# chathurawidanage/harp

Measured on AMD Instinct MI355X. Metric: sec/iteration K-means (N=1e8, d=100, K=1e4), lower is better.
Workload: dtype bf16; 1 GPU; model=kmeans-allreduce, N=100000000, d=100, K=10000, global_batch=100000000, parallelism=dp1

## Files before the change

csrc/kmeans_resolve.hip:

```cpp
#include "common.h"

namespace {

constexpr int KR_RUN = 2048;

template <int KS>
__global__ __launch_bounds__(64) __attribute__((amdgpu_waves_per_eu(3))) void kmeans_resolve_rowsum_kernel(
    const __bf16* __restrict__ X, long ldx, const __bf16* __restrict__ Cm2, const int* __restrict__ perm,
    const int* __restrict__ start, int NG, long n, int* __restrict__ labels, float* __restrict__ sums, int ld) {
  constexpr int DP = KS * 16;
  constexpr int NCB = (DP + 31) / 32;
  constexpr int STRE = NCB * 32 + 8;
  __shared__ __attribute__((aligned(16))) __bf16 tile[32 * STRE];
  __shared__ bf16x8 atile[KS * 64];
  const int lane = threadIdx.x;
  const int c = lane & 31, h = lane >> 5;
  const long j0 = (long)blockIdx.x * KR_RUN;
  if (j0 >= n) return;
  const long j1 = j0 + KR_RUN < n ? j0 + KR_RUN : n;

  for (int i = lane; i < 32 * STRE; i += 64) tile[i] = (__bf16)0.f;
  int lo = 0, hi = NG;
  while (hi - lo > 1) {
    const int mid = (lo + hi) >> 1;
    if (start[mid] <= j0) lo = mid; else hi = mid;
  }
  int k = lo;
  long kend = start[k + 1];
  int kloaded = -1;
  bool dirty = false;
  floatx16 S[NCB];
#pragma unroll
  for (int b = 0; b < NCB; ++b)
#pragma unroll
    for (int q = 0; q < 16; ++q) S[b][q] = 0.f;

  auto pos = [&](long jb) {
    const long j = jb + c;
    return j < j1 ? j : j1 - 1;
  };
  auto load_rows = [&](bf16x8 (&xf)[KS], int p) {
    const bf16x8* row = (const bf16x8*)(X + (long)p * ldx);
#pragma unroll
    for (int s = 0; s < KS; ++s) xf[s] = row[2 * s + h];
  };
  auto flush = [&](int kk) {
    float* o = sums + ((long)kk * 32 + 4 * h) * ld + c;
#pragma unroll
    for (int b = 0; b < NCB; ++b) {
#pragma unroll
      for (int q = 0; q < 16; ++q) {
        const int rq = (q & 3) + 8 * (q >> 2);
        if (32 * b + c < DP && S[b][q] != 0.f) atomicAdd(o + (long)rq * ld + 32 * b, S[b][q]);
        S[b][q] = 0.f;
      }
    }
  };

  bf16x8 xp[KS];
  int pp = perm[pos(j0)];
  int pn = perm[pos(j0 + 32)];
  load_rows(xp, pp);

  for (long jb = j0; jb < j1; jb += 32) {
    const long je = jb + 32 < j1 ? jb + 32 : j1;
    const long jj = jb + c;
    __syncthreads();
#pragma unroll
    for (int s = 0; s < KS; ++s) *(bf16x8*)(tile + c * STRE + (2 * s + h) * 8) = xp[s];
    const int pc = pp;
    if (jb + 32 < j1) load_rows(xp, pn);
    pp = pn;
    pn = perm[pos(jb + 64)];
    __syncthreads();
    long cur = jb;
    while (cur < je) {
      while (cur >= kend) {
        if (dirty) {
          flush(k);
          dirty = false;
        }
        ++k;
        kend = start[k + 1];
      }
      if (k != kloaded) {
        const bf16x8* arow = (const bf16x8*)(Cm2 + ((long)k * 32 + c) * DP);
#pragma unroll
        for (int s = 0; s < KS; ++s) atile[s * 64 + lane] = arow[2 * s + h];
        kloaded = k;
      }
      const long sub_end = kend < je ? kend : je;
      const bool mine = jj >= cur && jj < sub_end;
      floatx16 acc = {0.f, 0.f, 0.f, 0.f, 0.f, 0.f, 0.f, 0.f, 0.f, 0.f, 0.f, 0.f, 0.f, 0.f, 0.f, 0.f};
#pragma unroll
      for (int s = 0; s < KS; ++s) {
        acc = __builtin_amdgcn_mfma_f32_32x32x16_bf16(atile[s * 64 + lane],
                                                      *(const bf16x8*)(tile + c * STRE + (2 * s + h) * 8), acc, 0, 0, 0);
        __builtin_amdgcn_sched_barrier(0);
      }
      float m = acc[0];
      int mq = 0;
#pragma unroll
      for (int q = 1; q < 16; ++q)
        if (acc[q] < m) {
          m = acc[q];
          mq = q;
        }
      int row = (mq & 3) + 8 * (mq >> 2) + 4 * h;
      const float om = __shfl_xor(m, 32, 64);
      const int orow = __shfl_xor(row, 32, 64);
      if (om < m || (om == m && orow < row)) row = orow;
      if (mine && h == 0) labels[pc] = k * 32 + row;
      const int code = mine ? row : -1;
#pragma unroll
      for (int t = 0; t < 2; ++t) {
        bf16x8 oh;
#pragma unroll
        for (int j = 0; j < 8; ++j) {
          const int r0 = __builtin_amdgcn_readlane(code, 16 * t + j), r1 = __builtin_amdgcn_readlane(code, 16 * t + 8 + j);
          oh[j] = (__bf16)((h ? r1 : r0) == c ? 1.f : 0.f);
        }
        const __bf16* tp = tile + (16 * t + 8 * h) * STRE + c;
#pragma unroll
        for (int b = 0; b < NCB; ++b) {
          bf16x8 xt;
#pragma unroll
          for (int j = 0; j < 8; ++j) xt[j] = tp[j * STRE + 32 * b];
          S[b] = __builtin_amdgcn_mfma_f32_32x32x16_bf16(oh, xt, S[b], 0, 0, 0);
          __builtin_amdgcn_sched_barrier(0);
        }
      }
      dirty = true;
      cur = sub_end;
    }
  }
  if (dirty) flush(k);
}

template <int KS>
int launch_resolve(const void* X, long ldx, const void* Cm2, const int* perm, const int* start, int NG, long n,
                   int* labels, float* sums, int ld, hipStream_t s) {
  const long nblk = (n + KR_RUN - 1) / KR_RUN;
  kmeans_resolve_rowsum_kernel<KS><<<dim3((unsigned)nblk), dim3(64), 0, s>>>(
      (const __bf16*)X, ldx, (const __bf16*)Cm2, perm, start, NG, n, labels, sums, ld);
  return harp_launch_status();
}

}

HARP_EXPORT int harp_kmeans_resolve_rowsum(const void* X, long ldx, const void* Cm2, int dp, const int* perm,
                                           const int* start, int NG, long n, int* labels, float* sums, int ld,
                                           hipStream_t s) {
  if (n <= 0) return n == 0 ? HARP_OK : HARP_EBADARG;
  if (dp <= 0 || dp % 16 || dp > 128 || ldx < dp || ldx % 8 || ld < dp || NG <= 0 || !labels || !sums)
    return HARP_EBADARG;
  switch (dp / 16) {
    case 1: return launch_resolve<1>(X, ldx, Cm2, perm, start, NG, n, labels, sums, ld, s);
    case 2: return launch_resolve<2>(X, ldx, Cm2, perm, start, NG, n, labels, sums, ld, s);
    case 3: return launch_resolve<3>(X, ldx, Cm2, perm, start, NG, n, labels, sums, ld, s);
    case 4: return launch_resolve<4>(X, ldx, Cm2, perm, start, NG, n, labels, sums, ld, s);
    case 5: return launch_resolve<5>(X, ldx, Cm2, perm, start, NG, n, labels, sums, ld, s);
    case 6: return launch_resolve<6>(X, ldx, Cm2, perm, start, NG, n, labels, sums, ld, s);
    case 7: return launch_resolve<7>(X, ldx, Cm2, perm, start, NG, n, labels, sums, ld, s);
    case 8: return launch_resolve<8>(X, ldx, Cm2, perm, start, NG, n, labels, sums, ld, s);
    default: return HARP_EUNSUPPORTED;
  }
}
```

csrc/segsum.hip:

```cpp
#include "common.h"

namespace {

constexpr int SEG = 64;

__global__ __launch_bounds__(256) void label_hist_kernel(const int* __restrict__ lab, long n, int K, long chunk,
                                                         int* __restrict__ H) {
  extern __shared__ __attribute__((aligned(16))) int hist[];
  for (int k = threadIdx.x; k < K; k += blockDim.x) hist[k] = 0;
  __syncthreads();
  const long a = (long)blockIdx.x * chunk;
  long b = a + chunk;
  if (b > n) b = n;
  for (long i = a + threadIdx.x; i < b; i += blockDim.x) atomicAdd(&hist[lab[i]], 1);
  __syncthreads();
  int* row = H + (long)blockIdx.x * K;
  for (int k = threadIdx.x; k < K; k += blockDim.x) row[k] = hist[k];
}

__global__ void colscan1_kernel(int* __restrict__ H, int nchunks, int K, int* __restrict__ T) {
  const int k = blockIdx.x * blockDim.x + threadIdx.x;
  const int s = blockIdx.y;
  if (k >= K) return;
  const int c0 = s * SEG;
  int c1 = c0 + SEG;
  if (c1 > nchunks) c1 = nchunks;
  int run = 0;
  for (int c = c0; c < c1; ++c) {
    const int v = H[(long)c * K + k];
    H[(long)c * K + k] = run;
    run += v;
  }
  T[(long)s * K + k] = run;
}

__global__ void colscan2_kernel(int* __restrict__ T, int nseg, int K, int* __restrict__ counts) {
  const int k = blockIdx.x * blockDim.x + threadIdx.x;
  if (k >= K) return;
  int run = 0;
  for (int s = 0; s < nseg; ++s) {
    const int v = T[(long)s * K + k];
    T[(long)s * K + k] = run;
    run += v;
  }
  counts[k] = run;
}

__global__ __launch_bounds__(1024) void segscan_kernel(const int* __restrict__ counts, int K, int* __restrict__ start) {
  __shared__ int part[1024];
  const int per = (K + 1023) / 1024;
  const int a = threadIdx.x * per;
  int s = 0;
  for (int j = 0; j < per; ++j)
    if (a + j < K) s += counts[a + j];
  part[threadIdx.x] = s;
  __syncthreads();
  for (int off = 1; off < 1024; off <<= 1) {
    const int v = threadIdx.x >= off ? part[threadIdx.x - off] : 0;
    __syncthreads();
    part[threadIdx.x] += v;
    __syncthreads();
  }
  int run = threadIdx.x ? part[threadIdx.x - 1] : 0;
  for (int j = 0; j < per; ++j)
    if (a + j < K) {
      start[a + j] = run;
      run += counts[a + j];
    }
  if (threadIdx.x == 1023) start[K] = part[1023];
}

__device__ __forceinline__ int xcd_contiguous(unsigned b, unsigned nb) {
  const unsigned q = nb / 8, r = nb % 8, x = b % 8;
  return (int)((x < r ? x * (q + 1) : r * (q + 1) + (x - r) * q) + b / 8);
}

__global__ __launch_bounds__(256) void bucket_kernel(const int* __restrict__ lab, long n, int K, long chunk,
                                                     const int* __restrict__ H, const int* __restrict__ T,
                                                     const int* __restrict__ start, int* __restrict__ perm) {
  extern __shared__ __attribute__((aligned(16))) int cur[];
  const int c = xcd_contiguous(blockIdx.x, gridDim.x), s = c / SEG;
  for (int k = threadIdx.x; k < K; k += blockDim.x)
    cur[k] = start[k] + T[(long)s * K + k] + H[(long)c * K + k];
  __syncthreads();
  const long a = (long)c * chunk;
  long b = a + chunk;
  if (b > n) b = n;
  constexpr int U = 8;
  for (long i0 = a + threadIdx.x; i0 < b; i0 += (long)U * blockDim.x) {
    int l[U];
#pragma unroll
    for (int u = 0; u < U; ++u) {
      const long i = i0 + (long)u * blockDim.x;
      l[u] = i < b ? lab[i] : -1;
    }
#pragma unroll
    for (int u = 0; u < U; ++u)
      if (l[u] >= 0) perm[atomicAdd(&cur[l[u]], 1)] = (int)(i0 + (long)u * blockDim.x);
  }
}

template <int LPR, int RUN, int ROWS = 4>
__global__ __launch_bounds__(256) void rowsum_bf16_kernel(const __bf16* __restrict__ X, int dp, long ldx,
                                                          const int* __restrict__ perm,
                                                          const int* __restrict__ start, int K, long n,
                                                          float* __restrict__ sums, int ld) {
  constexpr int SPW = 64 / LPR;
  const int lane = threadIdx.x & 63;
  const int sl = lane % LPR;
  const long slot = ((long)blockIdx.x * blockDim.x + threadIdx.x) / LPR;
  const long j0 = slot * RUN;
  if (j0 >= n) return;
  long j1 = j0 + RUN;
  if (j1 > n) j1 = n;
  const bool active = sl * 8 < dp;
  int lo = 0, hi = K;
  while (hi - lo > 1) {
    const int mid = (lo + hi) >> 1;
    if (start[mid] <= j0) lo = mid; else hi = mid;
  }
  int k = lo;
  long kend = start[k + 1];
  float acc[8] = {0.f, 0.f, 0.f, 0.f, 0.f, 0.f, 0.f, 0.f};
  auto flush = [&](int kk) {
    if (active) {
      float* o = sums + (long)kk * ld + sl * 8;
#pragma unroll
      for (int e = 0; e < 8; ++e) {
        if (acc[e] != 0.f) atomicAdd(o + e, acc[e]);
        acc[e] = 0.f;
      }
    }
  };
  long j = j0;
  while (j < j1) {
    while (j >= kend) {
      flush(k);
      ++k;
      kend = start[k + 1];
    }
    long stop = kend < j1 ? kend : j1;
    for (; j + ROWS <= stop; j += ROWS) {
      bf16x8 v[ROWS];
      int pj[ROWS];
#pragma unroll
      for (int q = 0; q < ROWS; ++q) pj[q] = perm[j + q];
#pragma unroll
      for (int q = 0; q < ROWS; ++q) v[q] = active ? *(const bf16x8*)(X + (long)pj[q] * ldx + sl * 8) : bf16x8{};
#pragma unroll
      for (int q = 0; q < ROWS; q += 4)
#pragma unroll
        for (int e = 0; e < 8; ++e)
          acc[e] += ((float)v[q][e] + (float)v[q + 1][e]) + ((float)v[q + 2][e] + (float)v[q + 3][e]);
    }
    for (; j < stop; ++j) {
      if (active) {
        const bf16x8 v = *(const bf16x8*)(X + (long)perm[j] * ldx + sl * 8);
#pragma unroll
        for (int e = 0; e < 8; ++e) acc[e] += (float)v[e];
      }
    }
  }
  flush(k);
  (void)SPW;
}

template <int VEC, int RUN, int ROWS = 4>
__global__ __launch_bounds__(256) void rowsum_wide_bf16_kernel(const __bf16* __restrict__ X, int dp, long ldx,
                                                               const int* __restrict__ perm,
                                                               const int* __restrict__ start, int K, long n,
                                                               float* __restrict__ sums, int ld) {
  const int lane = threadIdx.x & 63;
  const long slot = ((long)blockIdx.x * blockDim.x + threadIdx.x) >> 6;
  const long j0 = slot * RUN;
  if (j0 >= n) return;
  long j1 = j0 + RUN;
  if (j1 > n) j1 = n;
  bool active[VEC];
#pragma unroll
  for (int c = 0; c < VEC; ++c) active[c] = (64 * c + lane) * 8 < dp;
  int lo = 0, hi = K;
  while (hi - lo > 1) {
    const int mid = (lo + hi) >> 1;
    if (start[mid] <= j0) lo = mid; else hi = mid;
  }
  int k = lo;
  long kend = start[k + 1];
  float acc[VEC][8];
#pragma unroll
  for (int c = 0; c < VEC; ++c)
#pragma unroll
    for (int e = 0; e < 8; ++e) acc[c][e] = 0.f;
  auto flush = [&](int kk) {
#pragma unroll
    for (int c = 0; c < VEC; ++c) {
      if (active[c]) {
        float* o = sums + (long)kk * ld + (64 * c + lane) * 8;
#pragma unroll
        for (int e = 0; e < 8; ++e) {
          if (acc[c][e] != 0.f) atomicAdd(o + e, acc[c][e]);
          acc[c][e] = 0.f;
        }
      }
    }
  };
  long j = j0;
  while (j < j1) {
    while (j >= kend) {
      flush(k);
      ++k;
      kend = start[k + 1];
    }
    const long stop = kend < j1 ? kend : j1;
    for (; j + ROWS <= stop; j += ROWS) {
      int pj[ROWS];
#pragma unroll
      for (int q = 0; q < ROWS; ++q) pj[q] = perm[j + q];
      bf16x8 v[ROWS][VEC];
#pragma unroll
      for (int q = 0; q < ROWS; ++q)
#pragma unroll
        for (int c = 0; c < VEC; ++c)
          v[q][c] = active[c] ? *(const bf16x8*)(X + (long)pj[q] * ldx + (64 * c + lane) * 8) : bf16x8{};
#pragma unroll
      for (int c = 0; c < VEC; ++c)
#pragma unroll
        for (int q = 0; q < ROWS; q += 4)
#pragma unroll
          for (int e = 0; e < 8; ++e)
            acc[c][e] += ((float)v[q][c][e] + (float)v[q + 1][c][e]) + ((float)v[q + 2][c][e] + (float)v[q + 3][c][e]);
    }
    for (; j < stop; ++j) {
      const long r = perm[j];
#pragma unroll
      for (int c = 0; c < VEC; ++c) {
        if (active[c]) {
          const bf16x8 v = *(const bf16x8*)(X + r * ldx + (64 * c + lane) * 8);
#pragma unroll
          for (int e = 0; e < 8; ++e) acc[c][e] += (float)v[e];
        }
      }
    }
  }
  flush(k);
}

}

HARP_EXPORT long harp_bucket_chunk(long n) {
  long c = 65536;
  while (c > 4096 && (n + c - 1) / c < 1536) c >>= 1;
  return c;
}

HARP_EXPORT long harp_bucket_workspace_ints(long n, int K) {
  const long chunk = harp_bucket_chunk(n);
  const long nch = (n + chunk - 1) / chunk;
  const long nseg = (nch + SEG - 1) / SEG;
  return nch * K + nseg * K + K + (K + 1) + n;
}

HARP_EXPORT int harp_bucket_labels(const int* lab, long n, int K, int* ws, long* start_off, long* perm_off,
                                   hipStream_t s) {
  if (n <= 0 || K <= 0 || K > 16384) return HARP_EBADARG;
  const long chunk = harp_bucket_chunk(n);
  const int nch = (int)((n + chunk - 1) / chunk);
  const int nseg = (nch + SEG - 1) / SEG;
  int* H = ws;
  int* T = H + (long)nch * K;
  int* counts = T + (long)nseg * K;
  int* start = counts + K;
  int* perm = start + K + 1;
  *start_off = start - ws;
  *perm_off = perm - ws;
  const size_t lds = (size_t)K * sizeof(int);
  label_hist_kernel<<<dim3(nch), dim3(256), lds, s>>>(lab, n, K, chunk, H);
  colscan1_kernel<<<dim3((K + 255) / 256, nseg), dim3(256), 0, s>>>(H, nch, K, T);
  colscan2_kernel<<<dim3((K + 255) / 256), dim3(256), 0, s>>>(T, nseg, K, counts);
  segscan_kernel<<<dim3(1), dim3(1024), 0, s>>>(counts, K, start);
  bucket_kernel<<<dim3(nch), dim3(256), lds, s>>>(lab, n, K, chunk, H, T, start, perm);
  return harp_launch_status();
}

HARP_EXPORT int harp_bucket_rowsum_bf16(const void* X, int dp, long ldx, const int* perm, const int* start, int K,
                                        long n, float* sums, int ld, hipStream_t s) {
  if (dp % 8 || dp > 1024 || ld < dp || ldx < dp || ldx % 8 || n <= 0) return n == 0 ? HARP_OK : HARP_EBADARG;
  const int lpr_min = dp / 8;
  const __bf16* Xb = (const __bf16*)X;
  constexpr int RUN = 256;
  auto grid = [&](int lpr) { return dim3((unsigned)(((n + RUN - 1) / RUN * lpr + 255) / 256)); };
  if (lpr_min <= 8) rowsum_bf16_kernel<8, RUN><<<grid(8), dim3(256), 0, s>>>(Xb, dp, ldx, perm, start, K, n, sums, ld);
  else if (lpr_min <= 16) rowsum_bf16_kernel<16, RUN, 8><<<grid(16), dim3(256), 0, s>>>(Xb, dp, ldx, perm, start, K, n, sums, ld);
  else if (lpr_min <= 32) rowsum_bf16_kernel<32, RUN><<<grid(32), dim3(256), 0, s>>>(Xb, dp, ldx, perm, start, K, n, sums, ld);
  else if (dp <= 512) rowsum_wide_bf16_kernel<1, RUN><<<grid(64), dim3(256), 0, s>>>(Xb, dp, ldx, perm, start, K, n, sums, ld);
  else rowsum_wide_bf16_kernel<2, RUN><<<grid(64), dim3(256), 0, s>>>(Xb, dp, ldx, perm, start, K, n, sums, ld);
  return harp_launch_status();
}
```

harp_amd/ops/_lib.py:

```python
from __future__ import annotations

import ctypes
import os
import threading

import torch

from .build import KERNEL_LIB, RUNTIME_LIB

_lock = threading.Lock()
_kern = None
_rt = None

c_int, c_long, c_float, c_void_p, c_ulonglong, c_double = (
    ctypes.c_int, ctypes.c_long, ctypes.c_float, ctypes.c_void_p, ctypes.c_ulonglong, ctypes.c_double)

_SIGNATURES = {
    "harp_kmeans_points_per_block": [c_int],
    "harp_kmeans_resident_blocks": [c_int, c_int],
    "harp_kmeans_set_resident_blocks": [c_int],
    "harp_kmeans_assign": [c_void_p, c_long, c_void_p, c_long, c_int, c_int, c_int, c_void_p, c_void_p, c_int,
                           c_void_p, c_void_p, c_int, c_void_p],
    "harp_kmeans_assign_wide": [c_void_p, c_long, c_void_p, c_long, c_int, c_int, c_int, c_int, c_void_p, c_int,
                                c_void_p],
    "harp_kmeans_wide_finish": [c_void_p, c_long, c_void_p, c_void_p, c_void_p, c_void_p],
    "harp_kmeans_normalize": [c_void_p, c_int, c_void_p, c_int, c_int, c_void_p, c_void_p],
    "harp_kmeans_prepare": [c_void_p, c_int, c_int, c_int, c_int, c_void_p, c_void_p, c_void_p],
    "harp_uniform_rows_bf16": [c_void_p, c_long, c_int, c_int, c_float, c_float, c_ulonglong, c_long, c_int,
                               c_void_p],
}


class NativeUnavailable(RuntimeError):
    pass


def _bind(lib, sigs):
    for name, args in sigs.items():
        try:
            fn = getattr(lib, name)
        except AttributeError:
            continue
        fn.argtypes = args
        fn.restype = c_int


def register(signatures: dict) -> None:
    _SIGNATURES.update(signatures)
    if _kern is not None:
        _bind(_kern, signatures)


def kernels():
    global _kern
    if _kern is not None:
        return _kern
    with _lock:
        if _kern is None:
            path = os.environ.get("HARP_KERNEL_LIB", KERNEL_LIB)
            if not os.path.exists(path):
                raise NativeUnavailable(
                    f"{path} not built: run `python -c 'import __graft_entry__ as g; g.build()'` "
                    "or `python -m harp_amd.ops.build`")
            try:
                lib = ctypes.CDLL(path, mode=ctypes.RTLD_GLOBAL)
            except OSError as e:
                raise NativeUnavailable(f"cannot load {path}: {e}") from e
            _bind(lib, _SIGNATURES)
            _kern = lib
    return _kern


def runtime():
    global _rt
    path = os.environ.get("HARP_RUNTIME_LIB", RUNTIME_LIB)
    if _rt is None and os.path.exists(path):
        with _lock:
            if _rt is None:
                _rt = ctypes.CDLL(path)
    return _rt


def available() -> bool:
    try:
        kernels()
        return True
    except NativeUnavailable:
        return False


def stream_ptr(device: torch.device | None = None) -> int:
    return torch.cuda.current_stream(device).cuda_stream


def ptr(t: torch.Tensor | None) -> int | None:
    return None if t is None else t.data_ptr()


def check(status: int, what: str) -> None:
    if status != 0:
        names = {1: "bad argument", 2: "launch failure", 3: "unsupported shape"}
        raise RuntimeError(f"{what}: native kernel returned {status} ({names.get(status, '?')})")


def use_native(t: torch.Tensor) -> bool:
    if t.device.type == "cuda":
        kernels()
        return True
    return False
```

harp_amd/ops/kmeans.py:

```python
from __future__ import annotations

import math
import os
from dataclasses import dataclass
from typing import Optional

import torch

from . import _lib, segment

KP_ALIGN = 128
ONES = 4
DEFAULT_VARIANT = 16
KEYLESS_VARIANT, KEYED_VARIANT = 16, 15
KEYLESS_MAX_DP = 128
RESOLVE_SPAN = 1 << 23


NARROW_MAX_DP = 256
WIDE_ALIGN = 64
WIDE_VARIANT = int(os.environ.get("HARP_KMEANS_WIDE_VARIANT", "0"))


def padded_dim(d: int) -> int:
    dp = (d + ONES + 15) // 16 * 16
    return dp if dp <= NARROW_MAX_DP else (d + ONES + WIDE_ALIGN - 1) // WIDE_ALIGN * WIDE_ALIGN


def padded_k(k: int) -> int:
    return (k + KP_ALIGN - 1) // KP_ALIGN * KP_ALIGN


def row_stride(dp: int) -> int:
    return (dp + 127) // 128 * 128


def pack_points(x: torch.Tensor, device: torch.device | str | None = None) -> torch.Tensor:
    device = torch.device(device) if device is not None else x.device
    n, d = x.shape
    dp = padded_dim(d)
    dt = torch.bfloat16 if device.type == "cuda" else torch.float32
    ld = row_stride(dp) if device.type == "cuda" else dp
    out = torch.zeros((n, ld), dtype=dt, device=device)
    out[:, :d] = x.to(device=device, dtype=dt)
    out[:, d:d + ONES] = 1.0
    return out[:, :dp]


def generate_points(n: int, d: int, lo: float = 0.0, hi: float = 1000.0, seed: int = 0,
                    device: torch.device | str = "cpu", row0: int = 0) -> torch.Tensor:
    device = torch.device(device)
    dp = padded_dim(d)
    if device.type == "cuda" and _lib.use_native(torch.empty(0, device=device)):
        ld = row_stride(dp)
        Xs = torch.empty((n, ld), dtype=torch.bfloat16, device=device)
        _lib.check(_lib.kernels().harp_uniform_rows_bf16(Xs.data_ptr(), n, d, ld, float(lo), float(hi),
                                                         seed & 0xFFFFFFFFFFFFFFFF, row0, 1,
                                                         _lib.stream_ptr(device)), "uniform_rows")
        return Xs[:, :dp]
    g = torch.Generator().manual_seed(seed * 1000003 + row0)
    x = torch.rand((n, d), generator=g, dtype=torch.float32) * (hi - lo) + lo
    return pack_points(x, device)


_SIDE: dict = {}


def pipeline_chunks(n: int, ppb: int) -> int:
    c = int(os.environ.get("HARP_KMEANS_CHUNKS", "1"))
    return max(1, min(c, n // (ppb * 256)))


def _side_stream(dev: torch.device) -> torch.cuda.Stream:
    s = _SIDE.get(dev)
    if s is None:
        s = _SIDE[dev] = torch.cuda.Stream(dev)
    return s


@dataclass
class CentroidOperand:
    Cm2: torch.Tensor
    cn: torch.Tensor
    K: int
    d: int


def prepare(c: torch.Tensor, dp: int, out: Optional[CentroidOperand] = None) -> CentroidOperand:
    K, d = c.shape
    Kp = padded_k(K)
    dev = c.device
    if out is None:
        dt = torch.bfloat16 if dev.type == "cuda" else torch.float32
        out = CentroidOperand(torch.empty((Kp, dp), dtype=dt, device=dev), torch.empty(Kp, dtype=torch.float32, device=dev), K, d)
    if _lib.use_native(c):
        cc = c.contiguous().float()
        _lib.check(_lib.kernels().harp_kmeans_prepare(cc.data_ptr(), K, d, Kp, dp, out.Cm2.data_ptr(),
                                                      out.cn.data_ptr(), _lib.stream_ptr(dev)), "kmeans_prepare")
        return out
    out.Cm2.zero_()
    out.Cm2[:K, :d] = -2.0 * c
    out.cn.fill_(1e38)
    out.cn[:K] = (c.double() ** 2).sum(1).float()
    return out


def resident_blocks(variant: int, dp: int) -> int:
    return _lib.kernels().harp_kmeans_resident_blocks(variant, dp // 16)


def set_resident_blocks(n: int) -> None:
    _lib.check(_lib.kernels().harp_kmeans_set_resident_blocks(n), "kmeans_set_resident_blocks")


def swept_k(op: "CentroidOperand") -> int:
    return min(op.Cm2.shape[0], (op.K + 31) // 32 * 32)


def _check_operands(X, op):
    assert X.dtype == torch.bfloat16 and X.stride(1) == 1 and X.stride(0) % 8 == 0 and op.Cm2.shape[1] == X.shape[1]


def _check_sums(sums, op, dev):
    assert sums.dtype == torch.float32 and sums.shape[1] >= op.d + 1 and sums.is_contiguous()
    assert sums.shape[0] >= op.Cm2.shape[0], "sums needs Kp (padded) rows"
    assert sums.device == dev


def _assign_wide(X, op, sums, labels, want_objective, obj_partial, min_dist):
    n, dp = X.shape
    dev = X.device
    lib = _lib.kernels()
    _check_operands(X, op)
    assert dp % WIDE_ALIGN == 0, f"wide rows need dp % {WIDE_ALIGN} == 0 (pack with padded_dim)"
    keys = torch.full((n,), -1, dtype=torch.int64, device=dev)
    _lib.check(lib.harp_kmeans_assign_wide(X.data_ptr(), X.stride(0), op.Cm2.data_ptr(), n, dp, swept_k(op),
                                           op.Cm2.shape[0], op.d, keys.data_ptr(), WIDE_VARIANT, _lib.stream_ptr(dev)),
               "kmeans_assign_wide")
    nblk = (n + 255) // 256
    if want_objective and (obj_partial is None or obj_partial.numel() < nblk):
        obj_partial = torch.empty(nblk, dtype=torch.float32, device=dev)
    _lib.check(lib.harp_kmeans_wide_finish(keys.data_ptr(), n, labels.data_ptr(),
                                           obj_partial.data_ptr() if want_objective else None,
                                           min_dist.data_ptr() if min_dist is not None else None,
                                           _lib.stream_ptr(dev)), "kmeans_wide_finish")
    if sums is not None:
        _check_sums(sums, op, dev)
        perm, start = segment.bucket_labels(labels, op.Cm2.shape[0])
        segment.bucket_rowsum(X, perm, start, sums)
    obj = obj_partial[:nblk].double().sum() if want_objective else None
    return labels, obj


def assign(X: torch.Tensor, op: CentroidOperand, sums: Optional[torch.Tensor] = None,
           labels: Optional[torch.Tensor] = None, want_objective: bool = True, variant: int = DEFAULT_VARIANT,
           obj_partial: Optional[torch.Tensor] = None, accumulate: str = "bucket",
           min_dist: Optional[torch.Tensor] = None):
    n, dp = X.shape
    dev = X.device
    if labels is None:
        labels = torch.empty(n, dtype=torch.int32, device=dev)
    if _lib.use_native(X):
        lib = _lib.kernels()
        if dp > NARROW_MAX_DP:
            if accumulate == "atomic":
                raise ValueError("accumulate='atomic' is only fused into the narrow kernel (dp <= "
                                 f"{NARROW_MAX_DP}); the wide path (dp = {dp}) accumulates by bucket")
            return _assign_wide(X, op, sums, labels, want_objective, obj_partial, min_dist)
        keyless = (variant == KEYLESS_VARIANT and dp <= KEYLESS_MAX_DP and sums is not None
                   and accumulate == "bucket" and min_dist is None)
        if variant == KEYLESS_VARIANT and not keyless:
            variant = KEYED_VARIANT
        if dp > 128:
            variant = 4
        elif variant in (14, 15) and dp // 16 == 5:
            variant = 13
        ppb = lib.harp_kmeans_points_per_block(variant)
        if ppb <= 0:
            raise ValueError(f"unknown kmeans kernel variant {variant}")
        nblk = (n + ppb - 1) // ppb
        if want_objective and (obj_partial is None or obj_partial.numel() < nblk):
            obj_partial = torch.empty(nblk, dtype=torch.float32, device=dev)
        if sums is not None:
            _check_sums(sums, op, dev)
        _check_operands(X, op)
        fused = sums if accumulate == "atomic" else None
        bucket = sums is not None and fused is None
        chunks = pipeline_chunks(n, ppb) if bucket else 1
        per = max(1, (nblk + chunks - 1) // chunks) * ppb
        side = _side_stream(dev) if chunks > 1 else None
        main = torch.cuda.current_stream(dev)
        for r0 in range(0, n, per):
            r1 = min(n, r0 + per)
            b0 = r0 // ppb
            st = lib.harp_kmeans_assign(X[r0].data_ptr(), X.stride(0), op.Cm2.data_ptr(), r1 - r0, dp,
                                        swept_k(op), op.d,
                                        labels[r0].data_ptr(), _lib.ptr(fused),
                                        fused.stride(0) if fused is not None else 0,
                                        obj_partial[b0].data_ptr() if want_objective else None,
                                        min_dist[r0].data_ptr() if min_dist is not None else None, variant,
                                        _lib.stream_ptr(dev))
            _lib.check(st, "kmeans_assign")
            if not bucket:
                continue

            def bucket_sum(lab, Xc):
                if keyless:
                    for s0 in range(0, lab.numel(), RESOLVE_SPAN):
                        ls, Xs = lab[s0:s0 + RESOLVE_SPAN], Xc[s0:s0 + RESOLVE_SPAN]
                        perm, start = segment.bucket_labels(ls, swept_k(op) // 32)
                        segment.resolve_rowsum(Xs, op.Cm2, perm, start, ls, sums)
                else:
                    perm, start = segment.bucket_labels(lab, op.Cm2.shape[0])
                    segment.bucket_rowsum(Xc, perm, start, sums)

            if side is None:
                bucket_sum(labels, X)
                continue
            side.wait_stream(main)
            with torch.cuda.stream(side):
                bucket_sum(labels[r0:r1], X[r0:r1])
        if side is not None:
            main.wait_stream(side)
        obj = obj_partial[:nblk].double().sum() if want_objective else None
        return labels, obj
    Xf = X.float()
    d = op.d
    x = Xf[:, :d]
    C = -0.5 * op.Cm2[: op.K, :d].float()
    dist = op.cn[: op.K].unsqueeze(0) - 2.0 * (x @ C.t())
    lab = dist.argmin(1)
    labels.copy_(lab.to(labels.dtype))
    if min_dist is not None:
        min_dist.copy_((dist.gather(1, lab[:, None])[:, 0] + (x * x).sum(1)).to(min_dist.dtype))
    if sums is not None:
        sums[:, : d + 1].index_add_(0, lab, Xf[:, : d + 1])
    obj = None
    if want_objective:
        xs = (x.double() ** 2).sum(1)
        obj = (dist.gather(1, lab[:, None])[:, 0].double() + xs).clamp_min(0).sum()
    return labels, obj


def normalize(sums: torch.Tensor, c: torch.Tensor, d: int, counts: Optional[torch.Tensor] = None) -> torch.Tensor:
    Kr = c.shape[0]
    if _lib.use_native(c):
        assert sums.is_contiguous() and c.is_contiguous()
        _lib.check(_lib.kernels().harp_kmeans_normalize(sums.data_ptr(), sums.stride(0), c.data_ptr(), Kr, d,
                                                        _lib.ptr(counts), _lib.stream_ptr(c.device)),
                   "kmeans_normalize")
        return c
    cnt = sums[:, d]
    m = cnt > 0
    c[m] = sums[m, :d] / cnt[m, None]
    if counts is not None:
        counts.copy_(cnt)
    return c
```

harp_amd/ops/segment.py:

```python
from __future__ import annotations

import ctypes
import os
from typing import Dict, Tuple

import torch

from . import _lib

_lib.register({
    "harp_bucket_chunk": [_lib.c_long],
    "harp_bucket_workspace_ints": [_lib.c_long, _lib.c_int],
    "harp_bucket_labels": [_lib.c_void_p, _lib.c_long, _lib.c_int, _lib.c_void_p, _lib.c_void_p, _lib.c_void_p,
                           _lib.c_void_p],
    "harp_bucket_rowsum_bf16": [_lib.c_void_p, _lib.c_int, _lib.c_long, _lib.c_void_p, _lib.c_void_p, _lib.c_int,
                                _lib.c_long, _lib.c_void_p, _lib.c_int, _lib.c_void_p],
    "harp_kmeans_resolve_rowsum": [_lib.c_void_p, _lib.c_long, _lib.c_void_p, _lib.c_int, _lib.c_void_p,
                                   _lib.c_void_p, _lib.c_int, _lib.c_long, _lib.c_void_p, _lib.c_void_p, _lib.c_int,
                                   _lib.c_void_p],
})
_WS: Dict[Tuple, torch.Tensor] = {}


def _lib_ret_long(fn):
    fn.restype = ctypes.c_long
    return fn


def bucket_labels(labels: torch.Tensor, K: int) -> Tuple[torch.Tensor, torch.Tensor]:
    n = labels.numel()
    if not _lib.use_native(labels):
        order = torch.argsort(labels.long(), stable=True)
        counts = torch.bincount(labels.long(), minlength=K)
        start = torch.zeros(K + 1, dtype=torch.int64)
        start[1:] = torch.cumsum(counts, 0)
        return order.to(torch.int32), start.to(torch.int32)
    lib = _lib.kernels()
    _lib_ret_long(lib.harp_bucket_workspace_ints)
    need = lib.harp_bucket_workspace_ints(n, K)
    stream = torch.cuda.current_stream(labels.device).cuda_stream
    key = (labels.device, n, K, stream)
    ws = _WS.get(key)
    if ws is None:
        ws = next((w for k, w in _WS.items() if k[0] == labels.device and k[3] == stream and w.numel() >= need),
                  None)
    if ws is None:
        for k in [k for k in _WS if k[3] == stream]:
            del _WS[k]
        ws = torch.empty(need, dtype=torch.int32, device=labels.device)
        _WS[key] = ws
    so, po = ctypes.c_long(0), ctypes.c_long(0)
    st = lib.harp_bucket_labels(labels.data_ptr(), n, K, ws.data_ptr(), ctypes.byref(so), ctypes.byref(po),
                                _lib.stream_ptr(labels.device))
    _lib.check(st, "bucket_labels")
    return ws[po.value:po.value + n], ws[so.value:so.value + K + 1]


SUM_SLICE = min(1024, max(8, int(os.environ.get("HARP_ROWSUM_SLICE", "1024")) // 8 * 8))


def bucket_rowsum(X: torch.Tensor, perm: torch.Tensor, start: torch.Tensor, out: torch.Tensor) -> torch.Tensor:
    K = start.numel() - 1
    if not _lib.use_native(X):
        idx = torch.repeat_interleave(torch.arange(K), (start[1:] - start[:-1]).long())
        out[:K, : X.shape[1]].index_add_(0, idx, X[perm.long()].float())
        return out
    assert X.dtype == torch.bfloat16 and X.stride(1) == 1 and out.dtype == torch.float32 and out.is_contiguous()
    for c0 in range(0, X.shape[1], SUM_SLICE):
        w = min(SUM_SLICE, X.shape[1] - c0)
        st = _lib.kernels().harp_bucket_rowsum_bf16(X[:, c0:].data_ptr(), w, X.stride(0), perm.data_ptr(),
                                                    start.data_ptr(), K, perm.numel(), out[:, c0:].data_ptr(),
                                                    out.stride(0), _lib.stream_ptr(X.device))
        _lib.check(st, "bucket_rowsum")
    return out


def resolve_rowsum(X: torch.Tensor, Cm2: torch.Tensor, perm: torch.Tensor, start: torch.Tensor,
                   labels: torch.Tensor, out: torch.Tensor) -> torch.Tensor:
    NG = start.numel() - 1
    dp = X.shape[1]
    assert X.dtype == torch.bfloat16 and X.stride(1) == 1 and out.dtype == torch.float32 and out.is_contiguous()
    assert Cm2.dtype == torch.bfloat16 and Cm2.is_contiguous() and Cm2.shape[1] == dp and Cm2.shape[0] >= 32 * NG
    assert out.shape[0] >= 32 * NG and labels.dtype == torch.int32 and labels.is_contiguous()
    assert labels.numel() == perm.numel() == X.shape[0]
    st = _lib.kernels().harp_kmeans_resolve_rowsum(X.data_ptr(), X.stride(0), Cm2.data_ptr(), dp, perm.data_ptr(),
                                                   start.data_ptr(), NG, perm.numel(), labels.data_ptr(),
                                                   out.data_ptr(), out.stride(0), _lib.stream_ptr(X.device))
    _lib.check(st, "kmeans_resolve_rowsum")
    return out
```

Before: 0.1323 s/iter.

## Bucket all spans in one pass and finish labels via rank gather

Replaces the Python loop over fixed-size spans, which launched a separate bucket and resolve pass per span, with one span-aware bucketing pipeline keyed by (span, group) and a single resolve launch. The resolve kernel now writes a per-sorted-position byte (row within group) instead of scattering int32 labels through perm. A new finish kernel gathers that byte by rank to build the final labels. The span size is enlarged so far fewer spans exist. This cuts launch count and repeated per-span histogram work and replaces random int32 label writes with coalesced byte writes. In exchange it adds a rank array write and a separate label-finishing pass.

```diff
diff --git a/csrc/kmeans_resolve.hip b/csrc/kmeans_resolve.hip
--- a/csrc/kmeans_resolve.hip
+++ b/csrc/kmeans_resolve.hip
@@ -7,7 +7,8 @@
 template <int KS>
 __global__ __launch_bounds__(64) __attribute__((amdgpu_waves_per_eu(3))) void kmeans_resolve_rowsum_kernel(
     const __bf16* __restrict__ X, long ldx, const __bf16* __restrict__ Cm2, const int* __restrict__ perm,
-    const int* __restrict__ start, int NG, long n, int* __restrict__ labels, float* __restrict__ sums, int ld) {
+    const int* __restrict__ start, int NG, int NB, long n, unsigned char* __restrict__ rowof,
+    float* __restrict__ sums, int ld) {
   constexpr int DP = KS * 16;
   constexpr int NCB = (DP + 31) / 32;
   constexpr int STRE = NCB * 32 + 8;
@@ -20,14 +21,15 @@
   const long j1 = j0 + KR_RUN < n ? j0 + KR_RUN : n;
 
   for (int i = lane; i < 32 * STRE; i += 64) tile[i] = (__bf16)0.f;
-  int lo = 0, hi = NG;
+  int lo = 0, hi = NB;
   while (hi - lo > 1) {
     const int mid = (lo + hi) >> 1;
     if (start[mid] <= j0) lo = mid; else hi = mid;
   }
   int k = lo;
   long kend = start[k + 1];
-  int kloaded = -1;
+  int g = k % NG;
+  int gloaded = -1;
   bool dirty = false;
   floatx16 S[NCB];
 #pragma unroll
@@ -44,8 +46,8 @@
 #pragma unroll
     for (int s = 0; s < KS; ++s) xf[s] = row[2 * s + h];
   };
-  auto flush = [&](int kk) {
-    float* o = sums + ((long)kk * 32 + 4 * h) * ld + c;
+  auto flush = [&](int gg) {
+    float* o = sums + ((long)gg * 32 + 4 * h) * ld + c;
 #pragma unroll
     for (int b = 0; b < NCB; ++b) {
 #pragma unroll
@@ -58,9 +60,8 @@
   };
 
   bf16x8 xp[KS];
-  int pp = perm[pos(j0)];
+  load_rows(xp, perm[pos(j0)]);
   int pn = perm[pos(j0 + 32)];
-  load_rows(xp, pp);
 
   for (long jb = j0; jb < j1; jb += 32) {
     const long je = jb + 32 < j1 ? jb + 32 : j1;
@@ -68,26 +69,27 @@
     __syncthreads();
 #pragma unroll
     for (int s = 0; s < KS; ++s) *(bf16x8*)(tile + c * STRE + (2 * s + h) * 8) = xp[s];
-    const int pc = pp;
     if (jb + 32 < j1) load_rows(xp, pn);
-    pp = pn;
     pn = perm[pos(jb + 64)];
     __syncthreads();
     long cur = jb;
     while (cur < je) {
-      while (cur >= kend) {
+      if (cur >= kend) {
         if (dirty) {
-          flush(k);
+          flush(g);
           dirty = false;
         }
-        ++k;
-        kend = start[k + 1];
-      }
-      if (k != kloaded) {
-        const bf16x8* arow = (const bf16x8*)(Cm2 + ((long)k * 32 + c) * DP);
+        do {
+          ++k;
+          kend = start[k + 1];
+        } while (cur >= kend);
+        g = k % NG;
+      }
+      if (g != gloaded) {
+        const bf16x8* arow = (const bf16x8*)(Cm2 + ((long)g * 32 + c) * DP);
 #pragma unroll
         for (int s = 0; s < KS; ++s) atile[s * 64 + lane] = arow[2 * s + h];
-        kloaded = k;
+        gloaded = g;
       }
       const long sub_end = kend < je ? kend : je;
       const bool mine = jj >= cur && jj < sub_end;
@@ -110,7 +112,7 @@
       const float om = __shfl_xor(m, 32, 64);
       const int orow = __shfl_xor(row, 32, 64);
       if (om < m || (om == m && orow < row)) row = orow;
-      if (mine && h == 0) labels[pc] = k * 32 + row;
+      if (mine && h == 0) rowof[jj] = (unsigned char)row;
       const int code = mine ? row : -1;
 #pragma unroll
       for (int t = 0; t < 2; ++t) {
@@ -134,35 +136,69 @@
       cur = sub_end;
     }
   }
-  if (dirty) flush(k);
+  if (dirty) flush(g);
 }
 
 template <int KS>
-int launch_resolve(const void* X, long ldx, const void* Cm2, const int* perm, const int* start, int NG, long n,
-                   int* labels, float* sums, int ld, hipStream_t s) {
+int launch_resolve(const void* X, long ldx, const void* Cm2, const int* perm, const int* start, int NG, int NB,
+                   long n, unsigned char* rowof, float* sums, int ld, hipStream_t s) {
   const long nblk = (n + KR_RUN - 1) / KR_RUN;
   kmeans_resolve_rowsum_kernel<KS><<<dim3((unsigned)nblk), dim3(64), 0, s>>>(
-      (const __bf16*)X, ldx, (const __bf16*)Cm2, perm, start, NG, n, labels, sums, ld);
+      (const __bf16*)X, ldx, (const __bf16*)Cm2, perm, start, NG, NB, n, rowof, sums, ld);
   return harp_launch_status();
 }
 
+template <bool VEC>
+__global__ __launch_bounds__(256) void kmeans_finish_labels_kernel(int* __restrict__ labels,
+                                                                   const int* __restrict__ rank,
+                                                                   const unsigned char* __restrict__ rowof, long n) {
+  const long p = ((long)blockIdx.x * 256 + threadIdx.x) * 4;
+  if (p >= n) return;
+  if (VEC && p + 4 <= n) {
+    const int4 r = *(const int4*)(rank + p);
+    int4 l = *(const int4*)(labels + p);
+    l.x = 32 * l.x + rowof[r.x];
+    l.y = 32 * l.y + rowof[r.y];
+    l.z = 32 * l.z + rowof[r.z];
+    l.w = 32 * l.w + rowof[r.w];
+    *(int4*)(labels + p) = l;
+  } else {
+    const long e = p + 4 < n ? p + 4 : n;
+    for (long i = p; i < e; ++i) labels[i] = 32 * labels[i] + rowof[rank[i]];
+  }
+}
+
+}
+
+HARP_EXPORT int harp_kmeans_finish_labels(int* labels, const int* rank, const unsigned char* rowof, long n,
+                                          hipStream_t s) {
+  if (n <= 0) return n == 0 ? HARP_OK : HARP_EBADARG;
+  if (!labels || !rank || !rowof || n >= (1L << 31)) return HARP_EBADARG;
+  const dim3 grid((unsigned)((n + 1023) / 1024));
+  if ((((uintptr_t)labels | (uintptr_t)rank) & 15) == 0)
+    kmeans_finish_labels_kernel<true><<<grid, dim3(256), 0, s>>>(labels, rank, rowof, n);
+  else
+    kmeans_finish_labels_kernel<false><<<grid, dim3(256), 0, s>>>(labels, rank, rowof, n);
+  return harp_launch_status();
 }
 
 HARP_EXPORT int harp_kmeans_resolve_rowsum(const void* X, long ldx, const void* Cm2, int dp, const int* perm,
-                                           const int* start, int NG, long n, int* labels, float* sums, int ld,
-                                           hipStream_t s) {
+                                           const int* start, int NG, int nspans, long n, unsigned char* rowof,
+                                           float* sums, int ld, hipStream_t s) {
   if (n <= 0) return n == 0 ? HARP_OK : HARP_EBADARG;
-  if (dp <= 0 || dp % 16 || dp > 128 || ldx < dp || ldx % 8 || ld < dp || NG <= 0 || !labels || !sums)
+  if (dp <= 0 || dp % 16 || dp > 128 || ldx < dp || ldx % 8 || ld < dp || NG <= 0 || nspans <= 0 ||
+      (long)nspans * NG >= (1L << 30) || n >= (1L << 31) || !rowof || !sums)
     return HARP_EBADARG;
+  const int NB = nspans * NG;
   switch (dp / 16) {
-    case 1: return launch_resolve<1>(X, ldx, Cm2, perm, start, NG, n, labels, sums, ld, s);
-    case 2: return launch_resolve<2>(X, ldx, Cm2, perm, start, NG, n, labels, sums, ld, s);
-    case 3: return launch_resolve<3>(X, ldx, Cm2, perm, start, NG, n, labels, sums, ld, s);
-    case 4: return launch_resolve<4>(X, ldx, Cm2, perm, start, NG, n, labels, sums, ld, s);
-    case 5: return launch_resolve<5>(X, ldx, Cm2, perm, start, NG, n, labels, sums, ld, s);
-    case 6: return launch_resolve<6>(X, ldx, Cm2, perm, start, NG, n, labels, sums, ld, s);
-    case 7: return launch_resolve<7>(X, ldx, Cm2, perm, start, NG, n, labels, sums, ld, s);
-    case 8: return launch_resolve<8>(X, ldx, Cm2, perm, start, NG, n, labels, sums, ld, s);
+    case 1: return launch_resolve<1>(X, ldx, Cm2, perm, start, NG, NB, n, rowof, sums, ld, s);
+    case 2: return launch_resolve<2>(X, ldx, Cm2, perm, start, NG, NB, n, rowof, sums, ld, s);
+    case 3: return launch_resolve<3>(X, ldx, Cm2, perm, start, NG, NB, n, rowof, sums, ld, s);
+    case 4: return launch_resolve<4>(X, ldx, Cm2, perm, start, NG, NB, n, rowof, sums, ld, s);
+    case 5: return launch_resolve<5>(X, ldx, Cm2, perm, start, NG, NB, n, rowof, sums, ld, s);
+    case 6: return launch_resolve<6>(X, ldx, Cm2, perm, start, NG, NB, n, rowof, sums, ld, s);
+    case 7: return launch_resolve<7>(X, ldx, Cm2, perm, start, NG, NB, n, rowof, sums, ld, s);
+    case 8: return launch_resolve<8>(X, ldx, Cm2, perm, start, NG, NB, n, rowof, sums, ld, s);
     default: return HARP_EUNSUPPORTED;
   }
 }
diff --git a/csrc/segsum.hip b/csrc/segsum.hip
--- a/csrc/segsum.hip
+++ b/csrc/segsum.hip
@@ -97,6 +97,74 @@
 #pragma unroll
     for (int u = 0; u < U; ++u)
       if (l[u] >= 0) perm[atomicAdd(&cur[l[u]], 1)] = (int)(i0 + (long)u * blockDim.x);
+  }
+}
+
+
+__global__ void colscan1_spans_kernel(int* __restrict__ H, int nchunks, int K, int seg, int* __restrict__ T) {
+  const int k = blockIdx.y * blockDim.x + threadIdx.x;
+  const int s = blockIdx.x;
+  if (k >= K) return;
+  const int c0 = s * seg;
+  int c1 = c0 + seg;
+  if (c1 > nchunks) c1 = nchunks;
+  int run = 0;
+  for (int c = c0; c < c1; ++c) {
+    const int v = H[(long)c * K + k];
+    H[(long)c * K + k] = run;
+    run += v;
+  }
+  T[(long)s * K + k] = run;
+}
+
+__global__ void colscan2_spans_kernel(int* __restrict__ T, int nseg, int sps, int K, int* __restrict__ counts) {
+  const int k = blockIdx.y * blockDim.x + threadIdx.x;
+  const int sp = blockIdx.x;
+  if (k >= K) return;
+  const int s0 = sp * sps;
+  int s1 = s0 + sps;
+  if (s1 > nseg) s1 = nseg;
+  int run = 0;
+  for (int s = s0; s < s1; ++s) {
+    const int v = T[(long)s * K + k];
+    T[(long)s * K + k] = run;
+    run += v;
+  }
+  counts[(long)sp * K + k] = run;
+}
+
+constexpr int SPAN_TPB = 1024;
+constexpr long SPAN_CHUNK = 16384;
+
+__global__ __launch_bounds__(SPAN_TPB) void bucket_spans_kernel(const int* __restrict__ lab, long n, int K,
+                                                                long chunk, int cps, int seg,
+                                                                const int* __restrict__ H, const int* __restrict__ T,
+                                                                const int* __restrict__ start, int* __restrict__ perm,
+                                                                int* __restrict__ rank) {
+  extern __shared__ __attribute__((aligned(16))) int cur[];
+  const int c = xcd_contiguous(blockIdx.x, gridDim.x), s = c / seg;
+  const int* st = start + (long)(c / cps) * K;
+  for (int k = threadIdx.x; k < K; k += blockDim.x) cur[k] = st[k] + T[(long)s * K + k] + H[(long)c * K + k];
+  __syncthreads();
+  const long a = (long)c * chunk;
+  long b = a + chunk;
+  if (b > n) b = n;
+  constexpr int U = 8;
+  for (long i0 = a + threadIdx.x; i0 < b; i0 += (long)U * blockDim.x) {
+    int l[U];
+#pragma unroll
+    for (int u = 0; u < U; ++u) {
+      const long i = i0 + (long)u * blockDim.x;
+      l[u] = i < b ? lab[i] : -1;
+    }
+#pragma unroll
+    for (int u = 0; u < U; ++u)
+      if (l[u] >= 0) {
+        const long i = i0 + (long)u * blockDim.x;
+        const int j = atomicAdd(&cur[l[u]], 1);
+        perm[j] = (int)i;
+        if (rank) rank[i] = j;
+      }
   }
 }
 
@@ -282,6 +350,65 @@
   return harp_launch_status();
 }
 
+namespace {
+
+struct SpanGeom {
+  long chunk;
+  int nch, cps, seg, nseg, sps, nspans;
+  long nb;
+};
+
+bool span_geom(long n, int K, long span, SpanGeom* g) {
+  if (n <= 0 || n >= (1L << 31) || K <= 0 || K > 16384 || span < 1024 || (span & (span - 1))) return false;
+  if (span > (1L << 31)) span = 1L << 31;
+  long chunk = harp_bucket_chunk(n) < SPAN_CHUNK ? harp_bucket_chunk(n) : SPAN_CHUNK;
+  if (chunk > span) chunk = span;
+  const long cps = span / chunk;
+  const long seg = cps < SEG ? cps : SEG;
+  const long nch = (n + chunk - 1) / chunk;
+  const long nspans = (n + span - 1) / span;
+  if (nspans * K >= (1L << 30)) return false;
+  g->chunk = chunk;
+  g->nch = (int)nch;
+  g->cps = (int)cps;
+  g->seg = (int)seg;
+  g->nseg = (int)((nch + seg - 1) / seg);
+  g->sps = (int)(cps / seg);
+  g->nspans = (int)nspans;
+  g->nb = nspans * K;
+  return true;
+}
+
+}
+
+HARP_EXPORT long harp_bucket_spans_workspace_ints(long n, int K, long span) {
+  SpanGeom g;
+  if (!span_geom(n, K, span, &g)) return 0;
+  return (long)g.nch * K + (long)g.nseg * K + g.nb + (g.nb + 1) + n;
+}
+
+HARP_EXPORT int harp_bucket_labels_spans(const int* lab, long n, int K, long span, int* ws, long* start_off,
+                                         long* perm_off, int* rank, hipStream_t s) {
+  SpanGeom g;
+  if (!lab || !ws || !span_geom(n, K, span, &g)) return HARP_EBADARG;
+  int* H = ws;
+  int* T = H + (long)g.nch * K;
+  int* counts = T + (long)g.nseg * K;
+  int* start = counts + g.nb;
+  int* perm = start + g.nb + 1;
+  *start_off = start - ws;
+  *perm_off = perm - ws;
+  const size_t lds = (size_t)K * sizeof(int);
+  const unsigned kb = (unsigned)((K + 255) / 256);
+  label_hist_kernel<<<dim3(g.nch), dim3(256), lds, s>>>(lab, n, K, g.chunk, H);
+  colscan1_spans_kernel<<<dim3(g.nseg, kb), dim3(256), 0, s>>>(H, g.nch, K, g.seg, T);
+  colscan2_spans_kernel<<<dim3(g.nspans, kb), dim3(256), 0, s>>>(T, g.nseg, g.sps, K, counts);
+  segscan_kernel<<<dim3(1), dim3(1024), 0, s>>>(counts, (int)g.nb, start);
+  bucket_spans_kernel<<<dim3(g.nch), dim3(SPAN_TPB), lds, s>>>(lab, n, K, g.chunk, g.cps, g.seg, H, T, start, perm,
+                                                             rank);
+  return harp_launch_status();
+}
+
 HARP_EXPORT int harp_bucket_rowsum_bf16(const void* X, int dp, long ldx, const int* perm, const int* start, int K,
                                         long n, float* sums, int ld, hipStream_t s) {
   if (dp % 8 || dp > 1024 || ld < dp || ldx < dp || ldx % 8 || n <= 0) return n == 0 ? HARP_OK : HARP_EBADARG;
diff --git a/harp_amd/ops/_lib.py b/harp_amd/ops/_lib.py
--- a/harp_amd/ops/_lib.py
+++ b/harp_amd/ops/_lib.py
@@ -28,6 +28,9 @@
     "harp_kmeans_prepare": [c_void_p, c_int, c_int, c_int, c_int, c_void_p, c_void_p, c_void_p],
     "harp_uniform_rows_bf16": [c_void_p, c_long, c_int, c_int, c_float, c_float, c_ulonglong, c_long, c_int,
                                c_void_p],
+    "harp_bucket_spans_workspace_ints": [c_long, c_int, c_long],
+    "harp_bucket_labels_spans": [c_void_p, c_long, c_int, c_long, c_void_p, c_void_p, c_void_p, c_void_p, c_void_p],
+    "harp_kmeans_finish_labels": [c_void_p, c_void_p, c_void_p, c_long, c_void_p],
 }
 
 
diff --git a/harp_amd/ops/kmeans.py b/harp_amd/ops/kmeans.py
--- a/harp_amd/ops/kmeans.py
+++ b/harp_amd/ops/kmeans.py
@@ -14,7 +14,7 @@
 DEFAULT_VARIANT = 16
 KEYLESS_VARIANT, KEYED_VARIANT = 16, 15
 KEYLESS_MAX_DP = 128
-RESOLVE_SPAN = 1 << 23
+RESOLVE_SPAN = 1 << 27
 
 
 NARROW_MAX_DP = 256
@@ -206,10 +206,10 @@
 
             def bucket_sum(lab, Xc):
                 if keyless:
-                    for s0 in range(0, lab.numel(), RESOLVE_SPAN):
-                        ls, Xs = lab[s0:s0 + RESOLVE_SPAN], Xc[s0:s0 + RESOLVE_SPAN]
-                        perm, start = segment.bucket_labels(ls, swept_k(op) // 32)
-                        segment.resolve_rowsum(Xs, op.Cm2, perm, start, ls, sums)
+                    ng = swept_k(op) // 32
+                    perm, start, rank, rowof = segment.bucket_labels_spans(lab, ng, RESOLVE_SPAN, want_rank=True)
+                    segment.resolve_rowsum(Xc, op.Cm2, perm, start, rowof, sums, NG=ng)
+                    segment.finish_labels(lab, rank, rowof)
                 else:
                     perm, start = segment.bucket_labels(lab, op.Cm2.shape[0])
                     segment.bucket_rowsum(Xc, perm, start, sums)
diff --git a/harp_amd/ops/segment.py b/harp_amd/ops/segment.py
--- a/harp_amd/ops/segment.py
+++ b/harp_amd/ops/segment.py
@@ -16,10 +16,11 @@
     "harp_bucket_rowsum_bf16": [_lib.c_void_p, _lib.c_int, _lib.c_long, _lib.c_void_p, _lib.c_void_p, _lib.c_int,
                                 _lib.c_long, _lib.c_void_p, _lib.c_int, _lib.c_void_p],
     "harp_kmeans_resolve_rowsum": [_lib.c_void_p, _lib.c_long, _lib.c_void_p, _lib.c_int, _lib.c_void_p,
-                                   _lib.c_void_p, _lib.c_int, _lib.c_long, _lib.c_void_p, _lib.c_void_p, _lib.c_int,
-                                   _lib.c_void_p],
+                                   _lib.c_void_p, _lib.c_int, _lib.c_int, _lib.c_long, _lib.c_void_p, _lib.c_void_p,
+                                   _lib.c_int, _lib.c_void_p],
 })
 _WS: Dict[Tuple, torch.Tensor] = {}
+_WS_SPANS: Dict[Tuple, torch.Tensor] = {}
 
 
 def _lib_ret_long(fn):
@@ -56,6 +57,43 @@
     return ws[po.value:po.value + n], ws[so.value:so.value + K + 1]
 
 
+def bucket_labels_spans(labels: torch.Tensor, K: int, span: int, want_rank: bool = False):
+    n = labels.numel()
+    nspans = (n + span - 1) // span
+    if not _lib.use_native(labels):
+        key = torch.arange(n, dtype=torch.int64) // span * K + labels.long()
+        order = torch.argsort(key, stable=True)
+        start = torch.zeros(nspans * K + 1, dtype=torch.int64)
+        start[1:] = torch.cumsum(torch.bincount(key, minlength=nspans * K), 0)
+        out = (order.to(torch.int32), start.to(torch.int32))
+        if want_rank:
+            rank = torch.empty(n, dtype=torch.int32)
+            rank[order] = torch.arange(n, dtype=torch.int32)
+            out += (rank, torch.empty(n, dtype=torch.uint8))
+        return out
+    assert labels.dtype == torch.int32 and labels.is_contiguous()
+    lib = _lib.kernels()
+    need = _lib_ret_long(lib.harp_bucket_spans_workspace_ints)(n, K, span)
+    if need <= 0:
+        raise ValueError(f"bucket_labels_spans: n = {n}, K = {K}, span = {span} (a power of two >= 1024, n < 2^31)")
+    base = (need + 3) // 4 * 4
+    total = base + (n + (n + 3) // 4 if want_rank else 0)
+    stream = torch.cuda.current_stream(labels.device).cuda_stream
+    key = (labels.device, stream)
+    ws = _WS_SPANS.get(key)
+    if ws is None or ws.numel() < total:
+        ws = _WS_SPANS[key] = torch.empty(total, dtype=torch.int32, device=labels.device)
+    rank = ws[base:base + n] if want_rank else None
+    so, po = ctypes.c_long(0), ctypes.c_long(0)
+    st = lib.harp_bucket_labels_spans(labels.data_ptr(), n, K, span, ws.data_ptr(), ctypes.byref(so), ctypes.byref(po),
+                                      _lib.ptr(rank), _lib.stream_ptr(labels.device))
+    _lib.check(st, "bucket_labels_spans")
+    out = (ws[po.value:po.value + n], ws[so.value:so.value + nspans * K + 1])
+    if want_rank:
+        out += (rank, ws[base + n:total].view(torch.uint8)[:n])
+    return out
+
+
 SUM_SLICE = min(1024, max(8, int(os.environ.get("HARP_ROWSUM_SLICE", "1024")) // 8 * 8))
 
 
@@ -76,15 +114,26 @@
 
 
 def resolve_rowsum(X: torch.Tensor, Cm2: torch.Tensor, perm: torch.Tensor, start: torch.Tensor,
-                   labels: torch.Tensor, out: torch.Tensor) -> torch.Tensor:
-    NG = start.numel() - 1
+                   rowof: torch.Tensor, out: torch.Tensor, NG: int | None = None) -> torch.Tensor:
+    NG = start.numel() - 1 if NG is None else NG
+    nspans = (start.numel() - 1) // NG
     dp = X.shape[1]
     assert X.dtype == torch.bfloat16 and X.stride(1) == 1 and out.dtype == torch.float32 and out.is_contiguous()
     assert Cm2.dtype == torch.bfloat16 and Cm2.is_contiguous() and Cm2.shape[1] == dp and Cm2.shape[0] >= 32 * NG
-    assert out.shape[0] >= 32 * NG and labels.dtype == torch.int32 and labels.is_contiguous()
-    assert labels.numel() == perm.numel() == X.shape[0]
+    assert out.shape[0] >= 32 * NG and rowof.dtype == torch.uint8 and rowof.is_contiguous()
+    assert rowof.numel() == perm.numel() == X.shape[0] and start.numel() == nspans * NG + 1
     st = _lib.kernels().harp_kmeans_resolve_rowsum(X.data_ptr(), X.stride(0), Cm2.data_ptr(), dp, perm.data_ptr(),
-                                                   start.data_ptr(), NG, perm.numel(), labels.data_ptr(),
+                                                   start.data_ptr(), NG, nspans, perm.numel(), rowof.data_ptr(),
                                                    out.data_ptr(), out.stride(0), _lib.stream_ptr(X.device))
     _lib.check(st, "kmeans_resolve_rowsum")
     return out
+
+
+def finish_labels(labels: torch.Tensor, rank: torch.Tensor, rowof: torch.Tensor) -> torch.Tensor:
+    assert labels.dtype == rank.dtype == torch.int32 and rowof.dtype == torch.uint8
+    assert labels.is_contiguous() and rank.is_contiguous() and rowof.is_contiguous()
+    assert labels.numel() == rank.numel() == rowof.numel()
+    st = _lib.kernels().harp_kmeans_finish_labels(labels.data_ptr(), rank.data_ptr(), rowof.data_ptr(),
+                                                  labels.numel(), _lib.stream_ptr(labels.device))
+    _lib.check(st, "kmeans_finish_labels")
+    return labels
```

Result: faster. 0.1307 s/iter (median of 6 runs) (-1.2%).
